# jrectorb/decagon

Measured on AMD Instinct MI355X. Metric: GCN-layer edges/sec + achieved HBM GB/s, 5-relation synthetic, 1/2/4/8 GPU, higher is better.
Workload: dtype f32; 1 GPU; S: main.py 5-relation / 10-matrix synthetic (reference-normalised, 105,974 nnz per relation set), 2 GCN layers d=64/32 + DEDICOM decoder B=512+512; nnz_per_layer_total=105974, parallelism=1 GPU, hipgraph=True, launch=one hipGraph per 30 steps, steps_per_graph=30

## Files before the change

decagon_amd/csrc/segspmm.hip:

```cpp
#include <cstddef>
#include <vector>

#include "common.h"
#include "peer.h"

constexpr int kSegU = 8;
constexpr int kSegUP = 4;
constexpr int kFsegU = 4;
constexpr int kFsegUP = 4;
constexpr int kSegMinNW = 1;
constexpr int kTabU = 4;
constexpr int kTabUP = 4;

namespace {

struct SegGroupK {
    const int32_t* rowptr;
    const int32_t* seg;
    const int32_t* vcol;
    const float* val;
    const int32_t* slab;
    const float* x;
    const float* w;
    float* out;
// ... 345 lines not shown
        }
        const int64_t o = (int64_t)(r0 + wave) * (4 * DOUT4) + 4 * lane;
        *reinterpret_cast<float4*>(T.out + o) = tot;
        if constexpr (PEER) dg::peer_store4(a.P, T.out, (uint32_t)T.n_rows * (16 * DOUT4), (uint32_t)o * 4, tot);
    }
#ifdef DG_FSEG_PROF
    asm volatile("s_waitcnt vmcnt(0)" ::: "memory");
    DG_FS_STAMP(6);
    if (lane == 0 && blockIdx.x < kFsProfMaxBlocks) {
        uint32_t xcc;
        asm volatile("s_getreg_b32 %0, hwreg(HW_REG_XCC_ID)" : "=s"(xcc));
        g_fs_prof[kFsForm][blockIdx.x][wave][7] = xcc;
    }
#endif
    if constexpr (PEER) dg::peer_arrive(a.P);
}

static_assert(sizeof(dg_tab_desc) == 64, "dg_tab_desc: one s_load_dwordx16");
static_assert(offsetof(dg_tab_desc, x) == 0, "dg_tab_desc layout");
static_assert(offsetof(dg_tab_desc, w) == 8, "dg_tab_desc layout");
static_assert(offsetof(dg_tab_desc, orow) == 16, "dg_tab_desc layout");
static_assert(offsetof(dg_tab_desc, cnt) == 24, "dg_tab_desc layout");
static_assert(offsetof(dg_tab_desc, x_ld) == 28, "dg_tab_desc layout");
static_assert(offsetof(dg_tab_desc, ovf) == 32, "dg_tab_desc layout");
static_assert(offsetof(dg_tab_desc, role) == 36, "dg_tab_desc layout");
static_assert(offsetof(dg_tab_desc, wr) == 40, "dg_tab_desc layout");
static_assert(offsetof(dg_tab_desc, aux_lo) == 44, "dg_tab_desc layout");
static_assert(offsetof(dg_tab_desc, aux_hi) == 48, "dg_tab_desc layout");
static_assert(offsetof(dg_tab_desc, gwaves) == 52, "dg_tab_desc layout");
static_assert(offsetof(dg_tab_desc, first_wave) == 56, "dg_tab_desc layout");
static_assert(offsetof(dg_tab_desc, reserved) == 60, "dg_tab_desc layout");
static_assert(kFsMaxRpb == DG_TAB_MAX_ROW_SLOTS && DG_TAB_ROLE_PROJ_SLOTS_BITS == DG_TAB_MAX_ROW_SLOTS,
              "dg_tab_desc: one mask bit per row slot");
template <bool PROJ, int U, int LP = 16>
__device__ __forceinline__ float4 tab_wave(const dg_tab_desc& D, const uint2 first, const uint2* __restrict__ ovf,
                                           float4* ybuf, const int S) {
    static_assert(LP == 16 || (LP == 8 && !PROJ), "tab_wave: 64-float rows, or 32-float plain sums");
    constexpr int G = dg::kWave / LP;
    [[maybe_unused]] constexpr int kFsForm = 1;
    const int lane = threadIdx.x & 63;
    float4 res = make_float4(0.f, 0.f, 0.f, 0.f);
    if (D.cnt > 0) {
        const float* xq = D.x + (lane % LP) * 4;
        const int sub = lane / LP;
        int vc = (int)first.x;
        int vb = (int)first.y;
        const uint2* nx = ovf + D.ovf;
        float4 acc = make_float4(0.f, 0.f, 0.f, 0.f);
        int bsz = S;
#pragma unroll 1
        for (int base = 0; base < D.cnt; base += bsz, bsz = 64) {
            const int n = min(bsz, D.cnt - base);
            const int eoff = vc * D.x_ld;
            const int vbits = vb;
            vc = 0;
            vb = 0;
            if (base + bsz < D.cnt) {
                const uint2 q = nx[lane];
                vc = (int)q.x;
                vb = (int)q.y;
                nx += 64;
            }
            constexpr int S = dg::kWave / G;
            static_assert(U >= 1 && U <= S && S % U == 0, "tab_wave: the unroll must divide the steps of a batch");
#pragma unroll
            for (int it = 0; it < S / U; ++it) {
                if (it * U * G >= n) break;
                int o[U];
                float w[U];
#pragma unroll
                for (int u = 0; u < U; ++u) {
                    const int m = it * U + u;
                    if constexpr (LP == 16) {
                        o[u] = row_bcast_rt(eoff, m);
                        w[u] = __int_as_float(row_bcast_rt(vbits, m));
                    } else {
                        const bool odd = (lane >> 3) & 1;
                        const int o0 = row_bcast_rt(eoff, m), o1 = row_bcast_rt(eoff, 8 + m);
                        const int w0 = row_bcast_rt(vbits, m), w1 = row_bcast_rt(vbits, 8 + m);
                        o[u] = odd ? o1 : o0;
                        w[u] = __int_as_float(odd ? w1 : w0);
                    }
                }
                float4 xv[U];
#pragma unroll
                for (int u = 0; u < U; ++u) {
                    const bool ok = (it * U + u) * G + sub < n;
                    xv[u] = ok ? *reinterpret_cast<const float4*>(xq + o[u]) : make_float4(0.f, 0.f, 0.f, 0.f);
                    if (!ok) w[u] = 0.f;
                }
#pragma unroll
                for (int u = 0; u < U; ++u) dg::fma4(acc, w[u], xv[u]);
            }
        }
        acc = dg::xor_sum4_from<LP>(acc);
#ifdef DG_FSEG_PROF
        if constexpr (PROJ) {
            asm volatile("s_waitcnt vmcnt(0) lgkmcnt(0)" ::: "memory");
            const int wave = __builtin_amdgcn_readfirstlane(threadIdx.x >> 6);
            DG_FS_STAMP(2);
        }
#endif
        if constexpr (PROJ) {
            const int ms = lane >> 3;
            const float4* w = reinterpret_cast<const float4*>(D.w) + (8 * ms) * 8 + (lane & 7);
            float4 wv[8];
#pragma unroll
            for (int i = 0; i < 8; ++i) wv[i] = w[8 * i];
            if (lane < 16) ybuf[lane] = acc;
            __builtin_amdgcn_wave_barrier();
            const float4 ya = ybuf[2 * ms];
            const float4 yb = ybuf[2 * ms + 1];
            float4 z = make_float4(0.f, 0.f, 0.f, 0.f);
            dg::fma4(z, ya.x, wv[0]);
            dg::fma4(z, ya.y, wv[1]);
            dg::fma4(z, ya.z, wv[2]);
            dg::fma4(z, ya.w, wv[3]);
            dg::fma4(z, yb.x, wv[4]);
            dg::fma4(z, yb.y, wv[5]);
            dg::fma4(z, yb.z, wv[6]);
            dg::fma4(z, yb.w, wv[7]);
            z = dg::xor_sum4_from<8>(z);
            res = z;
        } else {
            res = acc;
        }
    }
    return res;
}

template <int M>
__device__ __forceinline__ float xor_get_any(float x) {
    if constexpr (M == 0) {
        return x;
    } else {
        constexpr int LOW = M & -M;
        return xor_get_any<M - LOW>(dg::xor_get<LOW>(x));
    }
}
template <int M>
__device__ __forceinline__ float4 xor_get4_any(const float4& v) {
    return make_float4(xor_get_any<M>(v.x), xor_get_any<M>(v.y), xor_get_any<M>(v.z), xor_get_any<M>(v.w));
}
template <int W, int V, int SETS>
__device__ __forceinline__ void add_lane_sets(float4& tot, const float4& v, int n) {
    if constexpr (V < SETS) {
        if (V < n) dg::add4(tot, xor_get4_any<W * V>(v));
        add_lane_sets<W, V + 1, SETS>(tot, v, n);
    }
}

template <int W>
__device__ __forceinline__ float4 lds_ordered_sum(const float4 (*rows)[W], int K, int q) {
    float4 s = rows[0][q];
#pragma unroll 1
    for (int u = 1; u < K; ++u) dg::add4(s, rows[u][q]);
    return s;
}

template <int LP = 16>
__device__ __forceinline__ uint32_t slot_lane_offset(int lane, int S) {
    constexpr int G = dg::kWave / LP;
    const int q = S / G, m = lane & (LP - 1);
    return 8u * (uint32_t)((lane / LP) * q + (m < q ? m : q - 1));
}

__device__ __forceinline__ float4* tab_aux_row(const dg_tab_desc& D) {
    return reinterpret_cast<float4*>(((uint64_t)(uint32_t)D.aux_hi << 32) | (uint32_t)D.aux_lo);
}

__device__ __forceinline__ float4 load4_global(const float* p) {
    typedef float v4f __attribute__((ext_vector_type(4)));
    const v4f v = *(const v4f __attribute__((address_space(1)))*)(uintptr_t)p;
    return make_float4(v.x, v.y, v.z, v.w);
}

template <bool PROJ, int NW, bool PEER, int LP = 16, bool POST = false, bool DEC = false>
__global__ __launch_bounds__(64 * NW) void gcn_tab_kernel(const uint2* __restrict__ pairs,
                                                          const dg_tab_desc* __restrict__ desc,
                                                          const uint2* __restrict__ ovf, const int S,
                                                          const dg::PeerK P, const float* __restrict__ decG,
                                                          const float* __restrict__ decl) {
    static_assert(LP == 16 || (LP == 8 && !PROJ && !PEER), "gcn_tab_kernel: 32-float rows in the plain one-GPU form");
    static_assert(!POST || (LP == 16 && !PROJ && !PEER), "gcn_tab_kernel: the projecting tail follows a 64 -> 64 layer");
    static_assert(!DEC || (LP == 8 && !POST), "gcn_tab_kernel: the decoder's row operands follow the 32 -> 32 layer");
    constexpr int DOUT4 = PROJ ? 8 : LP;
    [[maybe_unused]] constexpr int kFsForm = (PROJ || LP == 8) ? 1 : 0;
    __shared__ float4 ybuf[NW][16];
    __shared__ float4 zbuf[NW][DOUT4];
    __shared__ float4 hbuf[POST ? kFsMaxRpb : 1][16];
    const int lane = threadIdx.x & 63;
    const int wave = __builtin_amdgcn_readfirstlane(threadIdx.x >> 6);
    const int64_t wi = (int64_t)blockIdx.x * NW + wave;
    DG_FS_STAMP(0);
    const dg_tab_desc D = desc[wi];
    uint2 first;
    asm volatile("global_load_dwordx2 %0, %1, %2\n\ts_waitcnt vmcnt(0)"
                 : "=&v"(first) : "v"(slot_lane_offset<LP>(lane, S)), "s"(pairs + wi * S) : "memory");
    asm volatile("" ::"s"(D.x), "s"(D.w), "s"(D.orow), "s"(D.cnt), "s"(D.x_ld), "s"(D.ovf), "s"(D.role), "s"(D.wr),
                 "s"(ovf));
    if constexpr (POST || DEC) asm volatile("" ::"s"(D.aux_lo), "s"(D.aux_hi));
#ifdef DG_FSEG_PROF
    asm volatile("s_waitcnt vmcnt(0) lgkmcnt(0)" ::: "memory");
#endif
    DG_FS_STAMP(1);
    if constexpr (!PROJ) DG_FS_STAMP(2);
    const int ms = lane >> 3;
    const float4 res = tab_wave<PROJ, PROJ ? kTabUP : kTabU, LP>(D, first, ovf, ybuf[wave], S);
    const bool djob = DEC && ((D.role >> DG_TAB_ROLE_DEC_BIT) & 1u) && D.orow != nullptr;
    float4 gv[DEC ? 4 : 1], lin, lout;
    if constexpr (DEC) {
        lin = lout = make_float4(1.f, 1.f, 1.f, 1.f);
        if (djob) {
            const float* gp = decG + 4 * ((4 * ms) * 8 + (lane & 7));
#pragma unroll
            for (int i = 0; i < 4; ++i) gv[i] = load4_global(gp + 4 * 8 * i);
            if (decl != nullptr) {
                lin = load4_global(decl + 4 * ms);
                lout = load4_global(decl + 4 * (lane & 7));
            }
        }
    }
    const bool pjob = POST && ((D.role >> DG_TAB_ROLE_PROJ_BIT) & 1u);
    float4 wv[POST ? 8 : 1];
    if constexpr (POST) {
        if (pjob) {
            const float* w = D.w + 4 * ((8 * ms) * 8 + (lane & 7));
#pragma unroll
            for (int i = 0; i < 8; ++i) wv[i] = load4_global(w + 4 * 8 * i);
        }
    }
#ifdef DG_FSEG_PROF
    asm volatile("s_waitcnt vmcnt(0) lgkmcnt(0)" ::: "memory");
#endif
    DG_FS_STAMP(3);
    if (lane < DOUT4) zbuf[wave][lane] = res;
    __syncthreads();
    DG_FS_STAMP(4);
    if (D.orow != nullptr) {
        constexpr int SETS = 64 / DOUT4;
        constexpr uint32_t kGw = (1u << DG_TAB_GWAVES_BITS) - 1u;
// ... 415 lines not shown
```

decagon_amd/engine.py:

```python
from __future__ import annotations

import heapq
import math
from dataclasses import dataclass
from typing import Callable, Dict, List, Optional, Sequence, Tuple

import numpy as np
import torch

from . import kernels, wavetable
from ._lib import DG_EPI_L2NORM, DG_EPI_RELU, DG_MAX_GROUPS
from .sparse import HostCSR, MergedCSR, chunk_segments, merge_chunks, merge_windows, staged_layout
from .tuning import knob

EdgeType = Tuple[int, int]


STAGED_MIN_RELS = knob("DG_STAGED_MIN_RELS", 32)
STAGED_MAX_COLS = 1024
STAGED_MAX_ROWS = 1022
STAGED_BINS = knob("DG_STAGED_BINS", 128)


def drop_tag(layer: int, group: int) -> int:
    return (layer << 16) | group


def stageable(n_rels: int, n_rows: int, n_cols: int) -> bool:
    return (knob("DG_STAGED", True) and n_rels >= STAGED_MIN_RELS
            and 0 < n_cols <= STAGED_MAX_COLS and 0 < n_rows <= STAGED_MAX_ROWS
            and kernels.staged_lds_bytes(n_rows, n_cols) <= kernels.STAGED_LDS_BYTES)


STAGED_TARGET_BLOCKS = knob("DG_STAGED_BLOCKS", 256)

WINDOW_MIN_ROWS = knob("DG_WINDOW_MIN_ROWS", 1024)
WINDOW_FULL_ROWS = 4096
N_WINDOWS = knob("DG_WINDOWS", 2)
FUSED_MAX_ROWS = knob("DG_FUSED_MAX_ROWS", 4096)
CONCURRENT_LAUNCHES = knob("DG_CONCURRENT", False)
STAGED_PROJ = knob("DG_STAGED_PROJ", True)
FUSED_SEG = knob("DG_FUSED_SEG", True)
SEG_FUSED = knob("DG_SEG_FUSED", True)
SEG_FUSED_MAX_ITEMS = 16
WAVE_TABLE = knob("DG_WAVE_TABLE", True)
TAB_BALANCE = knob("DG_TAB_BALANCE", 1)
L2_PREPROJECT = knob("DG_L2_PREPROJECT", True)
L2_PREPROJECT_SHARE = knob("DG_L2_PREPROJECT_SHARE", True)
STAGED_FIRST = knob("DG_STAGED_FIRST", True)
REASSOC_ROWS = knob("DG_REASSOC_ROWS", True)
SEG_ROWS_L1 = knob("DG_SEG_ROWS_L1", False)


def _epilogue(targets, d: int, flags: int, peer=None, push=None):
    if WAVE_TABLE:
        try:
            return kernels.PreparedEpilogueTab(targets, d, flags, peer=peer, push=push)
        except ValueError:
            pass
    return kernels.PreparedEpilogueMulti(targets, d, flags, peer=peer, push=push)


STAGED_VAR = knob("DG_STAGED_VAR", True)


def _lpt_bins(costs: np.ndarray, items: np.ndarray, n_bins: int, cap: int) -> List[List[int]]:
    order = items[np.argsort(-costs[items], kind="stable")]
    bins: List[List[int]] = [[] for _ in range(n_bins)]
    heap = [(0.0, b) for b in range(n_bins)]
    for it in order:
        full = []
        while True:
            load, b = heapq.heappop(heap)
            if len(bins[b]) < cap:
                break
            full.append((load, b))
        bins[b].append(int(it))
        heapq.heappush(heap, (load + float(costs[it]), b))
        for f in full:
            heapq.heappush(heap, f)
    return bins
# ... 103 lines not shown
        r0 += len(items)
    cost = np.where(B >= 0, c[np.maximum(B, 0)], np.nan)
    for _ in range(max_swaps):
        h = int(np.argmax(load))
        ch = cost[h]
        d = ch[None, :, None] - cost[:, None, :]
        with np.errstate(invalid="ignore"):
            new_max = np.maximum(load[h] - d, load[:, None, None] + d)
            gain = np.where((d > 0) & np.isfinite(d), load[h] - new_max, -np.inf)
        gain[h] = -np.inf
        k = int(np.argmax(gain))
        if not gain.flat[k] > 1e-9:
            break
        l, i, j = np.unravel_index(k, gain.shape)
        dd = d[l, i, j]
        B[h, i], B[l, j] = B[l, j], B[h, i]
        cost[h, i], cost[l, j] = cost[l, j], cost[h, i]
        load[h] -= dd
        load[l] += dd
    full = n_bins - 1 if cap[-1] < bin_size else n_bins
    by = list(np.argsort(-load[:full], kind="stable"))
    seq = []
    while by:
        seq.append(by.pop(0))
        if by:
            seq.append(by.pop())
    seq += list(range(full, n_bins))
    out = [int(i) for b in seq for i in B[b] if i >= 0]
    return np.asarray(out, np.int64)


def _tab_balance(d_in: int, d_out: int) -> bool:
    return TAB_BALANCE >= 2 or (TAB_BALANCE == 1 and d_in == d_out)


def _tab_groups_fit(tgts, d: int) -> bool:
    return all(len(gs) <= 64 // (d // 4) for _, _, gs, _ in tgts)


def choose_chunk(n_rels: int, n_rows: int, nnz: int, d: int, target_waves: int = 32768) -> int:
    if n_rels <= 1 or n_rows == 0:
        return max(1, n_rels)
    avg = nnz / float(n_rels * n_rows)
    chunk_traffic = max(1, math.ceil(4.0 * d / max(avg, 1e-9)))
    chunk_par = max(1, (n_rels * n_rows) // target_waves)
    chunk = chunk_par if chunk_traffic <= chunk_par else chunk_traffic
    return int(min(max(1, chunk), n_rels))


def row_slice(c: HostCSR, a: int, b: int) -> HostCSR:
    p0, p1 = int(c.rowptr[a]), int(c.rowptr[b])
    return HostCSR((c.rowptr[a:b + 1] - p0).astype(np.int32), c.col[p0:p1], c.val[p0:p1], (b - a, c.shape[1]))


@dataclass
class DeviceGroup:

    edge_type: EdgeType
    n_rows: int
    n_cols: int
    K: int
    rel_ids: np.ndarray
    chunk: int
    n_chunks: int
    rowptr: torch.Tensor
    vcol: torch.Tensor
# ... 348 lines not shown
                gemms.append(kernels.PreparedGemm(
                    hd, (n[j] * h1, h1, 1), W, (h1 * h2, h2, 1), self.proj[et], (n[j] * h2, h2, 1),
                    n[j], h2, h1, grp.n_rels, b_map=smap, b_batches=W.shape[0],
                    b_map_max=int(sids.max()) if smap is not None else None))
                continue
            gemms.append(kernels.PreparedGemm(
                self.hidden1[j], (0, h1, 1), W, (h1 * h2, h2, 1), self.proj[et], (n[j] * h2, h2, 1),
                n[j], h2, h1, grp.n_rels, b_map=grp.rel_map, b_batches=W.shape[0],
                b_map_max=int(grp.rel_ids.max()) if grp.rel_map is not None else None))
        self._gemm2 = drops + [kernels.PreparedGemmMulti(gemms[s:s + DG_MAX_GROUPS])
                               for s in range(0, len(gemms), DG_MAX_GROUPS)]
        self._layer2 = self._build_layer(self.proj, h2, False, f32,
                                         staged_proj={et: (self.hidden1[et[1]], w2.stacks[et])
                                                      for et in self.staged_proj},
                                         seg_w={et: (self.hidden1[et[1]], w2.stacks[et]) for et in self.seg_proj})

    def _fused_targets(self) -> List[int]:
        if self.flat_mode and (self.keep_sums or not self.row_block
                               or not getattr(self.shard, "fused_rows", False)):
            return []

        def rows(i):
            if i in self.row_block:
                return self.row_block[i][1] - self.row_block[i][0]
            return self.g.n_nodes[i]

        return [i for i, ets in self.targets.items()
                if (not self.flat_mode or i in self.row_block)
                and 0 < rows(i) <= FUSED_MAX_ROWS
                and all(self.g.groups[et].n_chunks == 1 and self.g.groups[et].n_rels > 0
                        and not self.g.groups[et].staged for et in ets)]

    def _preproject_fits(self, keep_sums: bool) -> bool:
        if not (L2_PREPROJECT and self.fused_seg and WAVE_TABLE and not keep_sums and self.drop_state is None
                and self.shard is None):
            return False
        order = list(self.targets)
        if any(et[1] not in self.targets for et in self.edge_types):
            return False
        if any(len(self.targets[i]) > 64 // (self.h1 // 4) for i in order):
            return False
        rels = {et: self.g.groups[et].n_rels for et in self.edge_types}
        waves_t = [sum(rels[et] for et in self.targets[i]) for i in order]
        sourced_t = [sum(k for et, k in rels.items() if et[1] == i) for i in order]
        return wavetable.tab_proj_fit(waves_t, sourced_t, _tab_balance(self.h1, self.h1), L2_PREPROJECT_SHARE)

    def _spec(self, et, x: torch.Tensor, out, d) -> kernels.RelGroupSpec:
        grp = self.g.groups[et]
        return kernels.RelGroupSpec(grp.rowptr, grp.vcol, grp.val, x, out, grp.n_rows, grp.n_chunks, d,
                                    grp.K * grp.n_cols, vcol_max=grp.vcol_max)

    def _seg_spec(self, et, x: torch.Tensor, out=None, w=None) -> kernels.SegSpec:
        grp = self.g.groups[et]
        if grp.seg is None and grp.seg2 is not None:
            rp, vc, vv, sg, ch, nc, vmax = grp.seg2
        else:
            rp, vc, vv, sg, ch, nc, vmax = grp.rowptr, grp.vcol, grp.val, grp.seg, grp.chunk, grp.n_chunks, grp.vcol_max
        return kernels.SegSpec(rp, sg, vc, vv, x, out, grp.n_rows, grp.n_cols, nc, ch, grp.n_rels, x.stride(-2),
                               grp.K * grp.n_cols, vcol_max=vmax, w=w, slab=grp.rel_map,
                               slab_max=int(grp.rel_ids.max()) if grp.n_rels else -1)

    def _seg_chunks(self, et) -> int:
        grp = self.g.groups[et]
        return grp.seg2[5] if (grp.seg is None and grp.seg2 is not None) else grp.n_chunks

    def _build_layer(self, xs: Dict[EdgeType, torch.Tensor], d, relu, f32, projs=(), staged_proj=None, seg_w=None,
                     post=None):
        g = self.g
        n = g.n_nodes
        outs = self.hidden1 if relu else self.embeddings
        launches: List[Callable[[], None]] = []
        fused_t = self.fused
        gathers = []
        if self.seg_mode and SEG_FUSED and all(sum(g.groups[et].n_rels for et in ets) <= SEG_FUSED_MAX_ITEMS
                                               for ets in self.targets.values()):
            seg_w = seg_w or {}
            tgts = []
            for i in self.targets:
                a, b, blk = self.row_block[i]
                pad = self._pad[i, 1 if relu else 2]
                r0 = self.shard.rank * blk
                gathers.append((pad, pad[r0:r0 + blk]))
                tgts.append((pad[r0:r0 + (b - a)], b - a,
                             [self._seg_spec(et, seg_w[et][0], None, seg_w[et][1]) if et in seg_w
                              else self._seg_spec(et, xs[et]) for et in self.targets[i]], relu))
            fused_peer = self._peer_fused(relu)
            d_in = self.h1 if seg_w else d
            if WAVE_TABLE and d_in == 64 and (d == 64 or seg_w) and _tab_groups_fit(tgts, d):
                launches.append(kernels.PreparedFusedTab(tgts, d_in, d, peer=fused_peer, balance=False))
            else:
                launches.append(kernels.PreparedFusedSeg(tgts, d_in, d, peer=fused_peer))
            self.launch_groups[id(launches[-1])] = [et for i in self.targets for et in self.targets[i]]
            if fused_peer is not None:
                gathers = []
            return _Layer(launches, None, False, self.allreduce, [], [], {}, self.side_stream, None, (), gathers,
                          self.allgather, self._peer_gather_all(gathers, relu))
        if self.fused_seg:
            seg_w = seg_w or {}
            tgts = [(outs[i], n[i], [self._seg_spec(et, seg_w[et][0], None, seg_w[et][1]) if et in seg_w
                                     else self._seg_spec(et, xs[et]) for et in self.targets[i]], relu)
                    for i in fused_t]
            d_in = self.h1 if seg_w else d
            if WAVE_TABLE and d_in == 64 and (d == 64 or seg_w) and _tab_groups_fit(tgts, d):
                pj = []
                for et, W2 in (post or {}).items():
                    grp = g.groups[et]
                    pj.append(kernels.TabProjSpec(fused_t.index(et[1]), W2, self.proj[et], grp.n_rels,
                                                  None if grp.rel_map is None else grp.rel_map.cpu().numpy()))
                launches.append(kernels.PreparedFusedTab(tgts, d_in, d, balance=_tab_balance(d_in, d), projs=pj,
                                                         share_proj=L2_PREPROJECT_SHARE))
            elif WAVE_TABLE and self.preproj and d_in == d == 32 and _tab_groups_fit(tgts, d):
                launches.append(kernels.PreparedFusedTab(tgts, d_in, d, balance=_tab_balance(d_in, d)))
                self._l2_tab = (tgts, d_in, d, _tab_balance(d_in, d), list(fused_t), launches[-1])
            else:
                launches.append(kernels.PreparedFusedSeg(tgts, d_in, d))
            self.launch_groups[id(launches[-1])] = [et for i in fused_t for et in self.targets[i]]
        elif fused_t:
            avg = max(g.groups[et].nnz / max(1, g.groups[et].n_rows) for i in fused_t for et in self.targets[i])
            max_groups = max(len(self.targets[i]) for i in fused_t)
            rows = sum(g.groups[self.targets[i][0]].n_rows for i in fused_t)
            cap = 16 // max_groups if self.row_block else 2
            wpg = 1 if rows >= 4096 else int(max(1, min(cap, 16 // max_groups, math.ceil(avg / 64.0))))
            if knob("DG_WPG", 0):
                wpg = max(1, min(knob("DG_WPG", 0), 16 // max_groups))
            pspecs = []
            for tgt_node, pj in projs:
                if tgt_node in fused_t:
                    pj.target = fused_t.index(tgt_node)
                    pspecs.append(pj)
            tgts = []
            for i in fused_t:
                out, rows_i = outs[i], n[i]
                if i in self.row_block:
                    a, b, blk = self.row_block[i]
                    pad = self._pad[i, 1 if relu else 2]
                    r0 = self.shard.rank * blk
                    out, rows_i = pad[r0:r0 + (b - a)], b - a
                    gathers.append((pad, pad[r0:r0 + blk]))
                tgts.append((out, rows_i, [self._spec(et, xs[et], None, d) for et in self.targets[i]], relu))
            launches.append(kernels.PreparedFused(tgts, d, pspecs, wpg))
            self.launch_groups[id(launches[-1])] = [et for i in fused_t for et in self.targets[i]]
        rest = [et for et in self.edge_types if et[0] not in fused_t]
        flags = DG_EPI_L2NORM | (DG_EPI_RELU if relu else 0)
        split_t = [i for i in self.targets if i in self.row_block and i not in fused_t]
        red = [et for et in rest if et[0] not in self.row_block]
        flat, views, send, sviews = None, {}, None, {}
# ... 180 lines not shown
            p()
        self._layer1.run()

    def run_layer2(self) -> None:
        for gm in self._gemm2:
            gm()
        self._layer2.run()

    def run(self) -> None:
        if self.peer is not None:
            self.peer.ensure_ok()
        self.run_layer1()
        self.run_layer2()
        self.runs += 1

    def attach_decoder_rows(self, node_type: int, G: torch.Tensor, l: Optional[torch.Tensor]):
        if not knob("DG_DEC_PREPROJECT", True):
            return None
        tab = getattr(self, "_l2_tab", None)
        if not self.preproj or tab is None or self.h2 != 32 or node_type not in tab[4]:
            return None
        if (G.dtype != torch.float32 or tuple(G.shape) != (32, 32) or not G.is_contiguous() or G.data_ptr() % 16
                or G.device != self.embeddings[node_type].device):
            return None
        if l is not None and (l.dtype != torch.float32 or tuple(l.shape) != (32,) or l.data_ptr() % 16
                              or l.device != G.device):
            return None
        key = (node_type, G.data_ptr(), None if l is None else l.data_ptr())
        if self._dec is not None:
            if self._dec["key"] != key:
                return None
            self._dec["users"] += 1
            return self._dec["Q"]
        tgts, d_in, d, balance, fused_t, plain = tab
        E = self.embeddings[node_type]
        Q = torch.zeros((E.shape[0], 32), dtype=torch.float32, device=E.device)
        launch = kernels.PreparedFusedTab(tgts, d_in, d, balance=balance,
                                          dec=kernels.TabDecSpec(fused_t.index(node_type), G, l, Q))
        self._swap_l2(plain, launch)
        self._dec = {"key": key, "Q": Q, "G": G, "l": l, "launch": launch, "users": 1, "runs": self.runs}
        return Q

    def release_decoder_rows(self, Q: torch.Tensor) -> None:
        if self._dec is None or self._dec["Q"] is not Q:
            return
        self._dec["users"] -= 1
        if self._dec["users"] > 0:
            return
        self._swap_l2(self._dec["launch"], self._l2_tab[5])
        self._dec_retired.append(self._dec)
        self._dec = None

    def decoder_rows_valid(self, Q: torch.Tensor) -> bool:
        return self._dec is not None and self._dec["Q"] is Q and self.runs > self._dec["runs"]

    def _swap_l2(self, old, new) -> None:
        L = self._layer2.launches
        L[L.index(old)] = new
        self.launch_groups[id(new)] = self.launch_groups[id(old)]

    def phases(self) -> List[Tuple[str, Callable[[], None]]]:
        out: List[Tuple[str, Callable[[], None]]] = []
        cur: List[Callable[[], None]] = []

        def close():
            if cur:
                fns = list(cur)
                out.append(("compute", lambda: [f() for f in fns]))
                cur.clear()

# ... 171 lines not shown
```

decagon_amd/kernels.py:

```python
from __future__ import annotations

import ctypes
from dataclasses import dataclass
from typing import Optional, Sequence, Tuple

import numpy as np
import torch

from . import _lib, wavetable
from .tuning import knob
from ._lib import (DgAdamSeg, DgEpiGroup, DgFusedTarget, DgGemmDesc, DgL2gGroup, DgProj, DgRelGroup,
                   DgStagedGroup, DgStagedProj, check)
from .wavetable import _balanced_waves, _proj_jobs, _tab_geometry, tab_proj_fit


def _stream_ptr(stream: Optional[torch.cuda.Stream] = None) -> int:
    s = torch.cuda.current_stream() if stream is None else stream
    return s.cuda_stream


def _dev(t: torch.Tensor, dtype: torch.dtype, what: str) -> torch.Tensor:
    if not isinstance(t, torch.Tensor):
        raise TypeError(f"{what}: expected a torch.Tensor, got {type(t).__name__}")
    if not t.is_cuda:
# ... 257 lines not shown
        self._keep = (specs, [t[0] for t in targets])
        self._tarr, self._ng, self._nt, self.d_in, self.d_out = tarr, len(specs), len(targets), d_in, d_out
        self._xchg = None
        if peer is not None:
            ex, slot = peer
            for out, *_ in targets:
                ex.offset(out)
            self._xchg = ctypes.byref(ex.xchg(slot))
            self._keep = self._keep + (ex,)
            self._fn = _lib.load().dg_gcn_fused_seg_peer_f32
        else:
            self._fn = _lib.load().dg_gcn_fused_seg_f32

    def __call__(self, stream=None) -> None:
        if self._xchg is not None:
            check(self._fn(self._garr, self._ng, self._tarr, self._nt, self.d_in, self.d_out, self._xchg,
                           _stream_ptr(stream)), "dg_gcn_fused_seg_peer_f32")
            return
        check(self._fn(self._garr, self._ng, self._tarr, self._nt, self.d_in, self.d_out, _stream_ptr(stream)),
              "dg_gcn_fused_seg_f32")


def _seg_data(s: SegSpec) -> wavetable.SegData:
    return wavetable.SegData(s.rowptr.cpu().numpy(), s.seg.cpu().numpy(), s.vcol.cpu().numpy(), s.val.cpu().numpy(),
                             None if s.slab is None else s.slab.cpu().numpy(), s.x.data_ptr(),
                             None if s.w is None else s.w.data_ptr(), None if s.out is None else s.out.data_ptr(),
                             s.x_ld, s.n_rows, s.n_cols, s.chunk, s.n_chunks, s.n_rels)


def _upload_table(owner, tab: wavetable.HostTable, dev) -> "_lib.DgWaveTable":
    owner._pairs = torch.from_numpy(tab.pairs).to(dev)
    owner._ovf = torch.from_numpy(tab.ovf).to(dev)
    owner.n_blocks, owner.nw, owner.slot_pairs = tab.n_blocks, tab.nw, tab.slot_pairs
    raw = torch.from_numpy(tab.desc.view(np.uint8).copy())
    owner._desc = torch.empty(raw.numel() + 64, dtype=torch.uint8, device=dev)
    off = (-owner._desc.data_ptr()) % 64
    owner._desc_v = owner._desc[off:off + raw.numel()]
    owner._desc_v.copy_(raw.to(dev))
    t = _lib.DgWaveTable()
    t.pairs, t.ovf, t.desc = owner._pairs.data_ptr(), owner._ovf.data_ptr(), owner._desc_v.data_ptr()
    t.n_blocks, t.nw, t.nw_stride, t.slot_pairs = tab.n_blocks, tab.nw, tab.stride, tab.slot_pairs
    return t


@dataclass
class TabProjSpec:

    target: int
    w: torch.Tensor
    out: torch.Tensor
    n_rels: int
    slab: Optional[Sequence[int]] = None


@dataclass
class TabDecSpec:

    target: int
    G: torch.Tensor
    l: Optional[torch.Tensor]
    out: torch.Tensor


class PreparedFusedTab(PreparedFusedSeg):

    def __init__(self, targets, d_in: int, d_out: int, peer=None, balance: bool = False,
                 projs: Sequence[TabProjSpec] = (), share_proj: bool = True, dec: Optional[TabDecSpec] = None):
        super().__init__(targets, d_in, d_out, peer=peer)
        specs = self._keep[0]
        narrow = d_in == d_out == 32 and all(s.w is None for s in specs) and peer is None
        self.dec = dec
        if dec is not None:
            _dev(dec.G, torch.float32, "G")
            _dev(dec.out, torch.float32, "Q")
            if dec.l is not None:
                _dev(dec.l, torch.float32, "l")
            if (not narrow or not 0 <= dec.target < len(targets) or tuple(dec.G.shape) != (32, 32)
                    or tuple(dec.out.shape) != (targets[dec.target][1], 32) or not dec.out.is_contiguous()
                    or not dec.G.is_contiguous() or (dec.l is not None and tuple(dec.l.shape) != (32,))
                    or dec.G.data_ptr() % 16 or dec.out.data_ptr() % 16
                    or (dec.l is not None and dec.l.data_ptr() % 16)):
                raise ValueError("dg_gcn_fused_tab_dec_f32: a 32 -> 32 launch, G [32, 32], l [32] or None, "
                                 "Q [target rows, 32], all 16-byte aligned")
        if not (wavetable._tab_shape(d_in, d_out, specs) or narrow):
            raise ValueError("dg_gcn_fused_tab_f32: d_in = d_out = 64, 64 -> 32 with weight stacks, or "
                             "d_in = d_out = 32 without an exchange")
        if any(len(gs) > 64 // (d_out // 4) for _, _, gs, _ in targets):
            raise ValueError("dg_gcn_fused_tab_f32: at most 64 / (d_out / 4) groups a target (one lane set each)")
        self.projs = list(projs)
        if self.projs and (d_in != 64 or d_out != 64 or peer is not None):
            raise ValueError("dg_gcn_fused_tab_post_f32: projection jobs follow a 64 -> 64 layer without an exchange")
        for pj in self.projs:
            _dev(pj.w, torch.float32, "w")
            _dev(pj.out, torch.float32, "P")
            K, rows = pj.w.shape[0], targets[pj.target][1]
            slabs = list(range(pj.n_rels)) if pj.slab is None else [int(x) for x in pj.slab[:pj.n_rels]]
            if (tuple(pj.w.shape[1:]) != (64, 32) or tuple(pj.out.shape) != (K, rows, 32) or len(slabs) != pj.n_rels
                    or any(not 0 <= x < K for x in slabs) or pj.out.data_ptr() % 16 or pj.w.data_ptr() % 16):
                raise ValueError("projection jobs: w [K, 64, 32], P [K, target rows, 32], slabs inside both")
        self.balance = balance
        data = {id(s): _seg_data(s) for s in specs}
        self._tab = _upload_table(self, wavetable.fused_table(
            [(out.data_ptr(), n_rows, [data[id(s)] for s in gs], relu) for out, n_rows, gs, relu in targets],
            d_in, d_out, balance=balance,
            projs=[wavetable.ProjData(pj.target, pj.w.data_ptr(), pj.out.data_ptr(), pj.n_rels, pj.slab)
                   for pj in self.projs],
            share_proj=share_proj, dec=None if dec is None else wavetable.DecData(dec.target, dec.out.data_ptr()),
            peer=peer is not None, slot=knob("DG_TAB_SLOT", 0)), specs[0].x.device)
        if dec is not None:
            self._keep = self._keep + (dec,)
            self._tfn, self._tname = _lib.load().dg_gcn_fused_tab_dec_f32, "dg_gcn_fused_tab_dec_f32"
        elif self._xchg is not None:
            self._tfn, self._tname = _lib.load().dg_gcn_fused_tab_peer_f32, "dg_gcn_fused_tab_peer_f32"
        elif self.projs:
            self._keep = self._keep + (self.projs,)
            self._tfn, self._tname = _lib.load().dg_gcn_fused_tab_post_f32, "dg_gcn_fused_tab_post_f32"
        else:
            self._tfn, self._tname = _lib.load().dg_gcn_fused_tab_f32, "dg_gcn_fused_tab_f32"

    def __call__(self, stream=None) -> None:
        if self.dec is not None:
            check(self._tfn(ctypes.byref(self._tab), self.d_in, self.d_out, self.dec.G.data_ptr(),
                            self.dec.l.data_ptr() if self.dec.l is not None else None, _stream_ptr(stream)),
                  self._tname)
        elif self._xchg is not None:
            check(self._tfn(ctypes.byref(self._tab), self.d_in, self.d_out, self._xchg, _stream_ptr(stream)),
                  self._tname)
        else:
            check(self._tfn(ctypes.byref(self._tab), self.d_in, self.d_out, _stream_ptr(stream)), self._tname)

    def seg_form(self, stream=None) -> None:
        PreparedFusedSeg.__call__(self, stream)


class PreparedSegTab(PreparedSeg):

    def __init__(self, specs: Sequence[SegSpec], d_in: int, d_out: int):
        super().__init__(specs, d_in, d_out)
        if not wavetable._tab_shape(d_in, d_out, specs):
            raise ValueError("dg_spmm_seg_tab_f32: d_in = d_out = 64, or 64 -> 32 with weight stacks")
        self._tab = _upload_table(self, wavetable.seg_table([_seg_data(s) for s in specs], d_in, d_out,
# ... 1176 lines not shown
```

decagon_amd/wavetable.py:

```python
from __future__ import annotations

from dataclasses import dataclass, field
from typing import List, NamedTuple, Optional, Sequence, Tuple

import numpy as np

DESC = np.dtype([("x", "<u8"), ("w", "<u8"), ("orow", "<u8"), ("cnt", "<i4"), ("x_ld", "<i4"), ("ovf", "<i4"),
                 ("role", "<u4"), ("wr", "<u4"), ("aux_lo", "<i4"), ("aux_hi", "<i4"), ("gwaves", "<i4"),
                 ("first_wave", "<i4"), ("reserved", "<i4")])
assert DESC.itemsize == 64

DG_TAB_ROLE_PROJ_BIT = 30
DG_TAB_ROLE_PROJ_SLOTS_SHIFT = 24
DG_TAB_ROLE_PROJ_SLOTS_BITS = 4
DG_TAB_ROLE_DEC_BIT = 29
DG_TAB_ROLE_SEG_WAVES_SHIFT = 8
DG_TAB_ROLE_SEG_WAVES_BITS = 8
DG_TAB_WR_GROUPS_BITS = 8
DG_TAB_WR_RELU_BIT = 8
DG_TAB_WR_SLOT_SHIFT = 16
DG_TAB_GWAVES_BITS = 4
DG_TAB_MAX_ROW_SLOTS = 4

PROJ_ROW_BYTES = 32 * 4
# ... 209 lines not shown


def _tab_shape(d_in: int, d_out: int, specs) -> bool:
    return d_in == 64 and (d_out == 64 or (d_out == 32 and all(s.w is not None for s in specs)))


def _tab_geometry(waves_t: Sequence[int], balance: bool) -> Tuple[int, int, List[int]]:
    nw = max([1] + list(waves_t))
    stride = 8 if nw <= 8 else 16
    if balance:
        nw = stride
    return nw, stride, [min(nw // max(1, w), DG_TAB_MAX_ROW_SLOTS) for w in waves_t]


def _proj_jobs(rows_present: Sequence[bool], n_rels: int, nw: int, share: bool = False):
    rpb = len(rows_present)
    if (n_rels if share else rpb * n_rels) > nw:
        return None
    jobs: List[Optional[Tuple[Tuple[int, ...], int]]] = [None] * nw
    order = list(range(rpb, nw)) + list(range(min(rpb, nw)))
    present = tuple(slot for slot in range(rpb) if rows_present[slot])
    if share:
        todo = [(present, k) for k in range(n_rels)] if present else []
    else:
        todo = [((slot,), k) for slot in present for k in range(n_rels)]
    for w, job in zip(order, todo):
        jobs[w] = job
    return jobs


def tab_proj_fit(waves_t: Sequence[int], sourced_t: Sequence[int], balance: bool, share: bool = False) -> bool:
    nw, _, rpbs = _tab_geometry(waves_t, balance)
    return all(_proj_jobs([True] * rpb, k, nw, share) is not None for rpb, k in zip(rpbs, sourced_t))


def _split_even(n: int, parts: int) -> List[Tuple[int, int]]:
    q, rem = divmod(n, parts)
    out, a = [], 0
    for p in range(parts):
        e = a + q + (1 if p < rem else 0)
        out.append((a, e))
        a = e
    return out


def _balanced_waves(tb: "_WaveTable", gs, nr, r: int, slots: int, proj: bool):
    if proj:
        jobs = [(gl, k) for gl in range(len(gs)) for k in range(nr[gl])]
        sizes = [tb.seg_len(gs[gl], k, r) for gl, k in jobs]
    else:
        jobs = [(gl, None) for gl in range(len(gs))]
        sizes = [sum(tb.seg_len(gs[gl], k, r) for k in range(nr[gl])) for gl in range(len(gs))]
    if len(jobs) > slots:
        raise ValueError(f"{len(jobs)} jobs for {slots} wave slots")
    parts = [1] * len(jobs)
    for _ in range(slots - len(jobs)):
        j = max(range(len(jobs)), key=lambda x: (-(-sizes[x] // parts[x]), -x))
        if sizes[j] <= parts[j]:
            break
        parts[j] += 1
    waves = [[] for _ in gs]
    for (gl, k), n, p in zip(jobs, sizes, parts):
        if k is not None:
            waves[gl] += [[(k, a, e)] for a, e in _split_even(n, p)]
            continue
        lens = [tb.seg_len(gs[gl], kk, r) for kk in range(nr[gl])]
        starts = np.cumsum([0] + lens)
        for a, e in _split_even(n, p):
            pieces = []
            for kk in range(nr[gl]):
                lo, hi = max(a, starts[kk]), min(e, starts[kk + 1])
                if lo < hi:
                    pieces.append((kk, int(lo - starts[kk]), int(hi - starts[kk])))
            waves[gl].append(pieces)
    return waves


def _mark_dec_rows(desc: np.ndarray, plan, stride: int, target: int, n_rows: int, q_ptr: int) -> int:
    done = 0
    for b, (t, r0, rpb) in enumerate(plan):
        if t != target:
            continue
        for w in range(rpb):
            if r0 + w >= n_rows:
                continue
            i = b * stride + w
            desc["role"][i] |= np.uint32(encode_role(dec=True))
            desc["aux_lo"][i], desc["aux_hi"][i] = split_addr(q_ptr + (r0 + w) * PROJ_ROW_BYTES)
            done += 1
    return done


def fused_table(targets, d_in: int, d_out: int, balance: bool = False, projs: Sequence[ProjData] = (),
                share_proj: bool = True, dec: Optional[DecData] = None, peer: bool = False,
                slot: int = 0) -> HostTable:
    specs = [s for _, _, gs, _ in targets for s in gs]
    proj = d_out != d_in
    waves_t = [sum(s.n_rels for s in gs) for _, _, gs, _ in targets]
    nw, stride, rpbs = _tab_geometry(waves_t, balance)
    plan = []
    for t, (_, n_rows, _, _) in enumerate(targets):
        plan += [(t, r0, rpbs[t]) for r0 in range(0, n_rows, rpbs[t])]
    tb = _WaveTable(specs, len(plan) * stride, proj, lp=d_in // 4)
    d = tb.desc
    g_first = np.cumsum([0] + [len(gs) for _, _, gs, _ in targets])
    for b, (t, r0, rpb) in enumerate(plan):
        out, n_rows, gspecs, relu = targets[t]
        gc = len(gspecs)
        nr = [s.n_rels for s in gspecs]
        gs = [int(g_first[t]) + gl for gl in range(gc)]
        per_row = nw // rpb if balance else waves_t[t]
        for slot_r in range(rpb):
            r = r0 + slot_r
            if r >= n_rows:
                continue
            if balance:
                waves = _balanced_waves(tb, gs, nr, r, per_row, proj)
            else:
                waves = [[[(k, 0, tb.seg_len(gs[gl], k, r))] for k in range(nr[gl])] for gl in range(gc)]
            w = slot_r * per_row
            for gl, wg in enumerate(waves):
                for pieces in wg:
                    tb.wave(b * stride + w, gs[gl], r, pieces)
                    w += 1
            i = b * stride + slot_r
            d["orow"][i] = out + r * d_out * 4
            d["wr"][i] = encode_wr(gc, relu, slot_r)
            d["aux_lo"][i], d["aux_hi"][i] = r * d_out * 4, n_rows * d_out * 4
            d["gwaves"][i] = encode_gwaves([len(wg) for wg in waves])
            d["first_wave"][i] = slot_r * per_row
        rels = [(pj, k) for pj in projs if pj.target == t for k in range(pj.n_rels)]
        if rels:
            jobs = _proj_jobs([r0 + s < n_rows for s in range(rpb)], len(rels), nw, share_proj)
            if jobs is None:
                raise ValueError(f"{rpb} rows x {len(rels)} projection jobs for {nw} wave slots")
            for w, job in enumerate(jobs):
                if job is None:
                    continue
                slots, (pj, k) = job[0], rels[job[1]]
                sl = k if pj.slab is None else int(pj.slab[k])
                i = b * stride + w
                d["role"][i] |= np.uint32(encode_role(proj_slots=slots))
                d["w"][i] = pj.w + sl * W_SLAB_BYTES
                d["aux_lo"][i], d["aux_hi"][i] = split_addr(pj.out + (sl * n_rows + r0) * PROJ_ROW_BYTES)
    if not plan and peer:
        raise ValueError("dg_gcn_fused_tab_peer_f32: the exchange needs at least one row a rank")
    if dec is not None:
        _mark_dec_rows(d, plan, stride, dec.target, targets[dec.target][1], dec.out)
    return tb.finish(len(plan), nw, stride, plan, slot)


def seg_table(specs: Sequence[SegData], d_in: int, d_out: int, slot: int = 0) -> HostTable:
    live = [g for g, s in enumerate(specs) if s.n_rows > 0 and s.n_rels > 0]
    nw = max([1] + [specs[g].chunk for g in live])
    stride = 8 if nw <= 8 else 16
    blocks = []
    for g in live:
        s = specs[g]
        rpb = nw // s.chunk
        row_blocks = -(-s.n_rows // rpb)
        items = s.n_chunks * row_blocks
        n_blocks = 8 * (-(-items // 8))
        per = n_blocks >> 3
        for lb in range(n_blocks):
            item = (lb & 7) * per + (lb >> 3)
            blocks.append(None if item >= items else (g, item // row_blocks, (item % row_blocks) * rpb, rpb))
# ... 20 lines not shown
```

Baseline: 15.60 billion edges/s.

## Pipeline table gathers through a load ring and add weighted row packing

In the plain-sum table kernel, the gather loop becomes a compile-time ring of outstanding loads that is three chunks deep. Loads for later edges are issued before earlier ones are folded in, and the next overflow batch is prefetched after the first issue, so gather latency is hidden. The LDS ordered sum is unrolled by four. On the host side, a weighted table plan packs rows into 16-wave blocks according to each row's segment lengths, with paired projection jobs, to balance work across waves. The price is more register pressure from the in-flight loads and a more complex table builder with new knobs.

```diff
diff --git a/decagon_amd/csrc/segspmm.hip b/decagon_amd/csrc/segspmm.hip
--- a/decagon_amd/csrc/segspmm.hip
+++ b/decagon_amd/csrc/segspmm.hip
@@ -401,10 +401,75 @@
 static_assert(offsetof(dg_tab_desc, reserved) == 60, "dg_tab_desc layout");
 static_assert(kFsMaxRpb == DG_TAB_MAX_ROW_SLOTS && DG_TAB_ROLE_PROJ_SLOTS_BITS == DG_TAB_MAX_ROW_SLOTS,
               "dg_tab_desc: one mask bit per row slot");
-template <bool PROJ, int U, int LP = 16>
+__device__ __forceinline__ float4 load4_global(const float* p) {
+    typedef float v4f __attribute__((ext_vector_type(4)));
+    const v4f v = *(const v4f __attribute__((address_space(1)))*)(uintptr_t)p;
+    return make_float4(v.x, v.y, v.z, v.w);
+}
+
+template <int LP>
+struct TabRing {
+    static constexpr int G = dg::kWave / LP, kC = 2, kD = 3, NC = (dg::kWave / G) / kC;
+    static_assert((dg::kWave / G) % kC == 0 && NC >= kD, "TabRing: chunks of a batch");
+    const float* xq;
+    int eoff, vbits, n, lane, safe;
+    float4 xv[kD][kC];
+
+    template <int M>
+    __device__ __forceinline__ int hand(int v) const {
+        if constexpr (LP == 16) {
+            return row_bcast<M>(v);
+        } else {
+            const int v0 = row_bcast<M>(v), v1 = row_bcast<8 + M>(v);
+            return ((lane >> 3) & 1) ? v1 : v0;
+        }
+    }
+    template <int M>
+    __device__ __forceinline__ bool has() const { return M * G + lane / LP < n; }
+    template <int C, int U = 0>
+    __device__ __forceinline__ void issue() {
+        if constexpr (U < kC) {
+            const int o = hand<C * kC + U>(eoff);
+            xv[C % kD][U] = load4_global(xq + (has<C * kC + U>() ? o : safe));
+            issue<C, U + 1>();
+        }
+    }
+    template <int C, int U = 0>
+    __device__ __forceinline__ void fold(float4& acc) const {
+        if constexpr (U < kC) {
+            const float w = __int_as_float(hand<C * kC + U>(vbits));
+            dg::fma4(acc, has<C * kC + U>() ? w : 0.f, xv[C % kD][U]);
+            fold<C, U + 1>(acc);
+        }
+    }
+    template <int C0, int C1>
+    __device__ __forceinline__ void fold_range(float4& acc) const {
+        if constexpr (C0 < C1) {
+            fold<C0>(acc);
+            fold_range<C0 + 1, C1>(acc);
+        }
+    }
+    template <int J>
+    __device__ __forceinline__ void run(float4& acc) {
+        constexpr int OLD = J >= kD - 1 ? J - (kD - 1) : 0;
+        if constexpr (J < NC) {
+            if (J * kC * G < n) {
+                issue<J>();
+                asm volatile("" : "+v"(acc.x), "+v"(acc.y), "+v"(acc.z), "+v"(acc.w)::"memory");
+                if constexpr (J >= kD - 1) fold<OLD>(acc);
+                run<J + 1>(acc);
+                return;
+            }
+        }
+        fold_range<OLD, J>(acc);
+    }
+};
+
+template <bool PROJ, int U, int LP = 16, bool OVL = false>
 __device__ __forceinline__ float4 tab_wave(const dg_tab_desc& D, const uint2 first, const uint2* __restrict__ ovf,
                                            float4* ybuf, const int S) {
     static_assert(LP == 16 || (LP == 8 && !PROJ), "tab_wave: 64-float rows, or 32-float plain sums");
+    static_assert(!(OVL && PROJ), "tab_wave: overlapped rounds in the plain sums");
     constexpr int G = dg::kWave / LP;
     [[maybe_unused]] constexpr int kFsForm = 1;
     const int lane = threadIdx.x & 63;
@@ -424,42 +489,52 @@
             const int vbits = vb;
             vc = 0;
             vb = 0;
-            if (base + bsz < D.cnt) {
-                const uint2 q = nx[lane];
-                vc = (int)q.x;
-                vb = (int)q.y;
-                nx += 64;
-            }
+            const auto prefetch = [&]() {
+                if (base + bsz < D.cnt) {
+                    const uint2 q = nx[lane];
+                    vc = (int)q.x;
+                    vb = (int)q.y;
+                    nx += 64;
+                }
+            };
+            if constexpr (!OVL) prefetch();
             constexpr int S = dg::kWave / G;
             static_assert(U >= 1 && U <= S && S % U == 0, "tab_wave: the unroll must divide the steps of a batch");
-#pragma unroll
-            for (int it = 0; it < S / U; ++it) {
-                if (it * U * G >= n) break;
-                int o[U];
-                float w[U];
-#pragma unroll
-                for (int u = 0; u < U; ++u) {
-                    const int m = it * U + u;
-                    if constexpr (LP == 16) {
-                        o[u] = row_bcast_rt(eoff, m);
-                        w[u] = __int_as_float(row_bcast_rt(vbits, m));
-                    } else {
-                        const bool odd = (lane >> 3) & 1;
-                        const int o0 = row_bcast_rt(eoff, m), o1 = row_bcast_rt(eoff, 8 + m);
-                        const int w0 = row_bcast_rt(vbits, m), w1 = row_bcast_rt(vbits, 8 + m);
-                        o[u] = odd ? o1 : o0;
-                        w[u] = __int_as_float(odd ? w1 : w0);
+            if constexpr (OVL) {
+                TabRing<LP> ring{xq, eoff, vbits, n, lane, __builtin_amdgcn_readfirstlane(eoff)};
+                ring.template issue<0>();
+                prefetch();
+                ring.template run<1>(acc);
+            } else {
+#pragma unroll
+                for (int it = 0; it < S / U; ++it) {
+                    if (it * U * G >= n) break;
+                    int o[U];
+                    float w[U];
+#pragma unroll
+                    for (int u = 0; u < U; ++u) {
+                        const int m = it * U + u;
+                        if constexpr (LP == 16) {
+                            o[u] = row_bcast_rt(eoff, m);
+                            w[u] = __int_as_float(row_bcast_rt(vbits, m));
+                        } else {
+                            const bool odd = (lane >> 3) & 1;
+                            const int o0 = row_bcast_rt(eoff, m), o1 = row_bcast_rt(eoff, 8 + m);
+                            const int w0 = row_bcast_rt(vbits, m), w1 = row_bcast_rt(vbits, 8 + m);
+                            o[u] = odd ? o1 : o0;
+                            w[u] = __int_as_float(odd ? w1 : w0);
+                        }
                     }
+                    float4 xv[U];
+#pragma unroll
+                    for (int u = 0; u < U; ++u) {
+                        const bool ok = (it * U + u) * G + sub < n;
+                        xv[u] = ok ? *reinterpret_cast<const float4*>(xq + o[u]) : make_float4(0.f, 0.f, 0.f, 0.f);
+                        if (!ok) w[u] = 0.f;
+                    }
+#pragma unroll
+                    for (int u = 0; u < U; ++u) dg::fma4(acc, w[u], xv[u]);
                 }
-                float4 xv[U];
-#pragma unroll
-                for (int u = 0; u < U; ++u) {
-                    const bool ok = (it * U + u) * G + sub < n;
-                    xv[u] = ok ? *reinterpret_cast<const float4*>(xq + o[u]) : make_float4(0.f, 0.f, 0.f, 0.f);
-                    if (!ok) w[u] = 0.f;
-                }
-#pragma unroll
-                for (int u = 0; u < U; ++u) dg::fma4(acc, w[u], xv[u]);
             }
         }
         acc = dg::xor_sum4_from<LP>(acc);
@@ -522,8 +597,22 @@
 template <int W>
 __device__ __forceinline__ float4 lds_ordered_sum(const float4 (*rows)[W], int K, int q) {
     float4 s = rows[0][q];
+    int u = 1;
 #pragma unroll 1
-    for (int u = 1; u < K; ++u) dg::add4(s, rows[u][q]);
+    for (; u + 4 <= K; u += 4) {
+        const float4 a = rows[u][q], b = rows[u + 1][q], c = rows[u + 2][q], d = rows[u + 3][q];
+        dg::add4(s, a);
+        dg::add4(s, b);
+        dg::add4(s, c);
+        dg::add4(s, d);
+    }
+    if (u + 2 <= K) {
+        const float4 a = rows[u][q], b = rows[u + 1][q];
+        dg::add4(s, a);
+        dg::add4(s, b);
+        u += 2;
+    }
+    if (u < K) dg::add4(s, rows[u][q]);
     return s;
 }
 
@@ -536,12 +625,6 @@
 
 __device__ __forceinline__ float4* tab_aux_row(const dg_tab_desc& D) {
     return reinterpret_cast<float4*>(((uint64_t)(uint32_t)D.aux_hi << 32) | (uint32_t)D.aux_lo);
-}
-
-__device__ __forceinline__ float4 load4_global(const float* p) {
-    typedef float v4f __attribute__((ext_vector_type(4)));
-    const v4f v = *(const v4f __attribute__((address_space(1)))*)(uintptr_t)p;
-    return make_float4(v.x, v.y, v.z, v.w);
 }
 
 template <bool PROJ, int NW, bool PEER, int LP = 16, bool POST = false, bool DEC = false>
@@ -575,7 +658,7 @@
     DG_FS_STAMP(1);
     if constexpr (!PROJ) DG_FS_STAMP(2);
     const int ms = lane >> 3;
-    const float4 res = tab_wave<PROJ, PROJ ? kTabUP : kTabU, LP>(D, first, ovf, ybuf[wave], S);
+    const float4 res = tab_wave<PROJ, PROJ ? kTabUP : kTabU, LP, !PROJ>(D, first, ovf, ybuf[wave], S);
     const bool djob = DEC && ((D.role >> DG_TAB_ROLE_DEC_BIT) & 1u) && D.orow != nullptr;
     float4 gv[DEC ? 4 : 1], lin, lout;
     if constexpr (DEC) {
diff --git a/decagon_amd/engine.py b/decagon_amd/engine.py
--- a/decagon_amd/engine.py
+++ b/decagon_amd/engine.py
@@ -47,6 +47,9 @@
 TAB_BALANCE = knob("DG_TAB_BALANCE", 1)
 L2_PREPROJECT = knob("DG_L2_PREPROJECT", True)
 L2_PREPROJECT_SHARE = knob("DG_L2_PREPROJECT_SHARE", True)
+TAB_WEIGHTED = knob("DG_TAB_WEIGHTED", 1)
+TAB_WEIGHTED_T64 = knob("DG_TAB_WEIGHTED_T64", 0)
+TAB_WEIGHTED_T32 = knob("DG_TAB_WEIGHTED_T32", 48)
 STAGED_FIRST = knob("DG_STAGED_FIRST", True)
 REASSOC_ROWS = knob("DG_REASSOC_ROWS", True)
 SEG_ROWS_L1 = knob("DG_SEG_ROWS_L1", False)
@@ -216,6 +219,12 @@
 
 def _tab_balance(d_in: int, d_out: int) -> bool:
     return TAB_BALANCE >= 2 or (TAB_BALANCE == 1 and d_in == d_out)
+
+
+def _tab_weighted(d_in: int, d_out: int) -> int:
+    if not (TAB_WEIGHTED and d_in == d_out and _tab_balance(d_in, d_out)):
+        return 0
+    return max(0, TAB_WEIGHTED_T64 if d_in == 64 else TAB_WEIGHTED_T32)
 
 
 def _tab_groups_fit(tgts, d: int) -> bool:
@@ -630,8 +639,8 @@
                         and not self.g.groups[et].staged for et in ets)]
 
     def _preproject_fits(self, keep_sums: bool) -> bool:
-        if not (L2_PREPROJECT and self.fused_seg and WAVE_TABLE and not keep_sums and self.drop_state is None
-                and self.shard is None):
+        self.tab_weighted = False
+        if not (self.fused_seg and WAVE_TABLE and not keep_sums and self.drop_state is None and self.shard is None):
             return False
         order = list(self.targets)
         if any(et[1] not in self.targets for et in self.edge_types):
@@ -641,7 +650,10 @@
         rels = {et: self.g.groups[et].n_rels for et in self.edge_types}
         waves_t = [sum(rels[et] for et in self.targets[i]) for i in order]
         sourced_t = [sum(k for et, k in rels.items() if et[1] == i) for i in order]
-        return wavetable.tab_proj_fit(waves_t, sourced_t, _tab_balance(self.h1, self.h1), L2_PREPROJECT_SHARE)
+        if not wavetable.tab_proj_fit(waves_t, sourced_t, _tab_balance(self.h1, self.h1), L2_PREPROJECT_SHARE):
+            return False
+        self.tab_weighted = wavetable.weighted_proj_fit(sourced_t, L2_PREPROJECT_SHARE)
+        return bool(L2_PREPROJECT)
 
     def _spec(self, et, x: torch.Tensor, out, d) -> kernels.RelGroupSpec:
         grp = self.g.groups[et]
@@ -706,10 +718,13 @@
                     pj.append(kernels.TabProjSpec(fused_t.index(et[1]), W2, self.proj[et], grp.n_rels,
                                                   None if grp.rel_map is None else grp.rel_map.cpu().numpy()))
                 launches.append(kernels.PreparedFusedTab(tgts, d_in, d, balance=_tab_balance(d_in, d), projs=pj,
-                                                         share_proj=L2_PREPROJECT_SHARE))
+                                                         share_proj=L2_PREPROJECT_SHARE,
+                                                         weighted=_tab_weighted(d_in, d) if self.tab_weighted else 0))
             elif WAVE_TABLE and self.preproj and d_in == d == 32 and _tab_groups_fit(tgts, d):
-                launches.append(kernels.PreparedFusedTab(tgts, d_in, d, balance=_tab_balance(d_in, d)))
-                self._l2_tab = (tgts, d_in, d, _tab_balance(d_in, d), list(fused_t), launches[-1])
+                weighted = _tab_weighted(d_in, d) if self.tab_weighted else 0
+                launches.append(kernels.PreparedFusedTab(tgts, d_in, d, balance=_tab_balance(d_in, d),
+                                                         weighted=weighted))
+                self._l2_tab = (tgts, d_in, d, _tab_balance(d_in, d), list(fused_t), launches[-1], weighted)
             else:
                 launches.append(kernels.PreparedFusedSeg(tgts, d_in, d))
             self.launch_groups[id(launches[-1])] = [et for i in fused_t for et in self.targets[i]]
@@ -956,10 +971,10 @@
                 return None
             self._dec["users"] += 1
             return self._dec["Q"]
-        tgts, d_in, d, balance, fused_t, plain = tab
+        tgts, d_in, d, balance, fused_t, plain, weighted = tab
         E = self.embeddings[node_type]
         Q = torch.zeros((E.shape[0], 32), dtype=torch.float32, device=E.device)
-        launch = kernels.PreparedFusedTab(tgts, d_in, d, balance=balance,
+        launch = kernels.PreparedFusedTab(tgts, d_in, d, balance=balance, weighted=weighted,
                                           dec=kernels.TabDecSpec(fused_t.index(node_type), G, l, Q))
         self._swap_l2(plain, launch)
         self._dec = {"key": key, "Q": Q, "G": G, "l": l, "launch": launch, "users": 1, "runs": self.runs}
diff --git a/decagon_amd/kernels.py b/decagon_amd/kernels.py
--- a/decagon_amd/kernels.py
+++ b/decagon_amd/kernels.py
@@ -313,6 +313,7 @@
     owner._pairs = torch.from_numpy(tab.pairs).to(dev)
     owner._ovf = torch.from_numpy(tab.ovf).to(dev)
     owner.n_blocks, owner.nw, owner.slot_pairs = tab.n_blocks, tab.nw, tab.slot_pairs
+    owner.host_plan = list(tab.plan)
     raw = torch.from_numpy(tab.desc.view(np.uint8).copy())
     owner._desc = torch.empty(raw.numel() + 64, dtype=torch.uint8, device=dev)
     off = (-owner._desc.data_ptr()) % 64
@@ -346,7 +347,8 @@
 class PreparedFusedTab(PreparedFusedSeg):
 
     def __init__(self, targets, d_in: int, d_out: int, peer=None, balance: bool = False,
-                 projs: Sequence[TabProjSpec] = (), share_proj: bool = True, dec: Optional[TabDecSpec] = None):
+                 projs: Sequence[TabProjSpec] = (), share_proj: bool = True, dec: Optional[TabDecSpec] = None,
+                 weighted: int = 0):
         super().__init__(targets, d_in, d_out, peer=peer)
         specs = self._keep[0]
         narrow = d_in == d_out == 32 and all(s.w is None for s in specs) and peer is None
@@ -379,7 +381,7 @@
             if (tuple(pj.w.shape[1:]) != (64, 32) or tuple(pj.out.shape) != (K, rows, 32) or len(slabs) != pj.n_rels
                     or any(not 0 <= x < K for x in slabs) or pj.out.data_ptr() % 16 or pj.w.data_ptr() % 16):
                 raise ValueError("projection jobs: w [K, 64, 32], P [K, target rows, 32], slabs inside both")
-        self.balance = balance
+        self.balance, self.weighted = balance, weighted
         data = {id(s): _seg_data(s) for s in specs}
         self._tab = _upload_table(self, wavetable.fused_table(
             [(out.data_ptr(), n_rows, [data[id(s)] for s in gs], relu) for out, n_rows, gs, relu in targets],
@@ -387,7 +389,7 @@
             projs=[wavetable.ProjData(pj.target, pj.w.data_ptr(), pj.out.data_ptr(), pj.n_rels, pj.slab)
                    for pj in self.projs],
             share_proj=share_proj, dec=None if dec is None else wavetable.DecData(dec.target, dec.out.data_ptr()),
-            peer=peer is not None, slot=knob("DG_TAB_SLOT", 0)), specs[0].x.device)
+            peer=peer is not None, slot=knob("DG_TAB_SLOT", 0), weighted=weighted), specs[0].x.device)
         if dec is not None:
             self._keep = self._keep + (dec,)
             self._tfn, self._tname = _lib.load().dg_gcn_fused_tab_dec_f32, "dg_gcn_fused_tab_dec_f32"
diff --git a/decagon_amd/wavetable.py b/decagon_amd/wavetable.py
--- a/decagon_amd/wavetable.py
+++ b/decagon_amd/wavetable.py
@@ -265,6 +265,62 @@
 def tab_proj_fit(waves_t: Sequence[int], sourced_t: Sequence[int], balance: bool, share: bool = False) -> bool:
     nw, _, rpbs = _tab_geometry(waves_t, balance)
     return all(_proj_jobs([True] * rpb, k, nw, share) is not None for rpb, k in zip(rpbs, sourced_t))
+
+
+WEIGHTED_STRIDE = 16
+
+
+def _weighted_slots(sizes: Sequence[int], T: int) -> int:
+    if len(sizes) > WEIGHTED_STRIDE:
+        raise ValueError(f"{len(sizes)} groups for {WEIGHTED_STRIDE} wave slots")
+    return min(max(sum(max(1, -(-int(n) // T)) for n in sizes), len(sizes)), WEIGHTED_STRIDE)
+
+
+def _weighted_max_rows(n_rels: int, share: bool) -> int:
+    for rows in range(DG_TAB_MAX_ROW_SLOTS, 0, -1):
+        if (-(-rows // 2) if share else rows) * n_rels <= WEIGHTED_STRIDE:
+            return rows
+    return 0
+
+
+def _proj_jobs_paired(rows_present: Sequence[bool], n_rels: int, nw: int, share: bool = True):
+    rpb = len(rows_present)
+    if not share:
+        return _proj_jobs(rows_present, n_rels, nw, False)
+    if -(-rpb // 2) * n_rels > nw:
+        return None
+    jobs: List[Optional[Tuple[Tuple[int, ...], int]]] = [None] * nw
+    order = list(range(rpb, nw)) + list(range(min(rpb, nw)))
+    todo = []
+    for s0 in range(0, rpb, 2):
+        present = tuple(s for s in range(s0, min(s0 + 2, rpb)) if rows_present[s])
+        if present:
+            todo += [(present, k) for k in range(n_rels)]
+    for w, job in zip(order, todo):
+        jobs[w] = job
+    return jobs
+
+
+def weighted_proj_fit(sourced_t: Sequence[int], share: bool = True) -> bool:
+    return all(_weighted_max_rows(k, share) >= 1 for k in sourced_t)
+
+
+def _weighted_plan(tb: "_WaveTable", targets, g_first, T: int, max_rows: Sequence[int]):
+    plan, firsts = [], []
+    for t, (_, n_rows, gspecs, _) in enumerate(targets):
+        gs = [int(g_first[t]) + gl for gl in range(len(gspecs))]
+        r0, cur = 0, []
+        for r in range(n_rows):
+            w = _weighted_slots([sum(tb.seg_len(g, k, r) for k in range(s.n_rels)) for g, s in zip(gs, gspecs)], T)
+            if cur and (sum(cur) + w > WEIGHTED_STRIDE or len(cur) >= max_rows[t]):
+                plan.append((t, r0, len(cur)))
+                firsts.append(cur)
+                r0, cur = r, []
+            cur.append(w)
+        if cur:
+            plan.append((t, r0, len(cur)))
+            firsts.append(cur)
+    return plan, [[(sum(c[:i]), c[i]) for i in range(len(c))] for c in firsts]
 
 
 def _split_even(n: int, parts: int) -> List[Tuple[int, int]]:
@@ -326,17 +382,29 @@
 
 def fused_table(targets, d_in: int, d_out: int, balance: bool = False, projs: Sequence[ProjData] = (),
                 share_proj: bool = True, dec: Optional[DecData] = None, peer: bool = False,
-                slot: int = 0) -> HostTable:
+                slot: int = 0, weighted: int = 0) -> HostTable:
     specs = [s for _, _, gs, _ in targets for s in gs]
     proj = d_out != d_in
     waves_t = [sum(s.n_rels for s in gs) for _, _, gs, _ in targets]
-    nw, stride, rpbs = _tab_geometry(waves_t, balance)
-    plan = []
-    for t, (_, n_rows, _, _) in enumerate(targets):
-        plan += [(t, r0, rpbs[t]) for r0 in range(0, n_rows, rpbs[t])]
+    g_first = np.cumsum([0] + [len(gs) for _, _, gs, _ in targets])
+    row_slots = None
+    if weighted:
+        if weighted < 1 or not balance or proj or peer:
+            raise ValueError("a weighted table: balanced plain sums (d_in == d_out) without an exchange, T >= 1")
+        nw = stride = WEIGHTED_STRIDE
+        max_rows = [_weighted_max_rows(sum(pj.n_rels for pj in projs if pj.target == t), share_proj)
+                    for t in range(len(targets))]
+        if not all(max_rows):
+            raise ValueError(f"one row's projection jobs for {nw} wave slots")
+        plan, row_slots = _weighted_plan(_WaveTable(specs, 0, proj, lp=d_in // 4), targets, g_first, weighted,
+                                         max_rows)
+    else:
+        nw, stride, rpbs = _tab_geometry(waves_t, balance)
+        plan = []
+        for t, (_, n_rows, _, _) in enumerate(targets):
+            plan += [(t, r0, rpbs[t]) for r0 in range(0, n_rows, rpbs[t])]
     tb = _WaveTable(specs, len(plan) * stride, proj, lp=d_in // 4)
     d = tb.desc
-    g_first = np.cumsum([0] + [len(gs) for _, _, gs, _ in targets])
     for b, (t, r0, rpb) in enumerate(plan):
         out, n_rows, gspecs, relu = targets[t]
         gc = len(gspecs)
@@ -347,11 +415,14 @@
             r = r0 + slot_r
             if r >= n_rows:
                 continue
+            first = slot_r * per_row
+            if row_slots is not None:
+                first, per_row = row_slots[b][slot_r]
             if balance:
                 waves = _balanced_waves(tb, gs, nr, r, per_row, proj)
             else:
                 waves = [[[(k, 0, tb.seg_len(gs[gl], k, r))] for k in range(nr[gl])] for gl in range(gc)]
-            w = slot_r * per_row
+            w = first
             for gl, wg in enumerate(waves):
                 for pieces in wg:
                     tb.wave(b * stride + w, gs[gl], r, pieces)
@@ -361,10 +432,11 @@
             d["wr"][i] = encode_wr(gc, relu, slot_r)
             d["aux_lo"][i], d["aux_hi"][i] = r * d_out * 4, n_rows * d_out * 4
             d["gwaves"][i] = encode_gwaves([len(wg) for wg in waves])
-            d["first_wave"][i] = slot_r * per_row
+            d["first_wave"][i] = first
         rels = [(pj, k) for pj in projs if pj.target == t for k in range(pj.n_rels)]
         if rels:
-            jobs = _proj_jobs([r0 + s < n_rows for s in range(rpb)], len(rels), nw, share_proj)
+            jobs = (_proj_jobs_paired if weighted else _proj_jobs)([r0 + s < n_rows for s in range(rpb)], len(rels),
+                                                                   nw, share_proj)
             if jobs is None:
                 raise ValueError(f"{rpb} rows x {len(rels)} projection jobs for {nw} wave slots")
             for w, job in enumerate(jobs):
```

Result: faster. 16.61 billion edges/s (median of 6 runs) (+6.5%).
